# secondlaw-ai/skyrim

Measured on AMD Instinct MI355X. Metric: 6-h forecast steps/sec on 721x1440 state, 1/2/4/8 MI355X; per-channel max rel-err vs ref, higher is better.
Workload: dtype f16; 1 GPU; Pangu 6-h autoregressive rollout, 721x1440x69 state (13 levels x 5 vars + 4 surface), random-init weights (64 M params), state resident in HBM, 1 ensemble membe; parallelism=single GPU, members=1, finite=True, rounding=compensated, term_plan=0x66f

## Files before the change

### skyrim_amd/csrc/attention.hip

```cpp
#include <cstdlib>
#include "gemm_dma.h"
#include "launchers.h"

namespace skp {

__device__ __forceinline__ int attn_key(int f, int row) {
    return f < 8 ? 32 * (f >> 1) + 8 * (row >> 2) + 4 * (f & 1) + (row & 3) : 128 + row;
}

__device__ __forceinline__ void attn_softmax_pv(f32x4 (&s)[9], const uint4 (&vf)[2][5], f32x4 (&o)[2], f32x4& osum) {
    typedef f16 T;
    const float LOG2E = 1.4426950408889634f;
    float mx = s[0][0];
#pragma unroll
    for (int f = 0; f < 9; ++f)
#pragma unroll
        for (int r = 0; r < 4; ++r) mx = fmaxf(mx, s[f][r]);
    mx = fmaxf(mx, __shfl_xor(mx, 16));
    mx = fmaxf(mx, __shfl_xor(mx, 32));
    const float mxl = mx * LOG2E;
#pragma unroll
    for (int f = 0; f < 9; ++f)
#pragma unroll
        for (int r = 0; r < 4; ++r) s[f][r] = __builtin_amdgcn_exp2f(__builtin_fmaf(s[f][r], LOG2E, -mxl));
    o[0] = f32x4{0.f, 0.f, 0.f, 0.f}; o[1] = f32x4{0.f, 0.f, 0.f, 0.f}; osum = f32x4{0.f, 0.f, 0.f, 0.f};
    const uint4 ones = make_uint4(0x3C003C00u, 0x3C003C00u, 0x3C003C00u, 0x3C003C00u);
#pragma unroll
    for (int kb = 0; kb < 5; ++kb) {
        float pv[8];
#pragma unroll
        for (int r = 0; r < 4; ++r) {
            pv[r] = s[2 * kb][r];
            pv[4 + r] = (kb < 4) ? s[(2 * kb + 1) % 9][r] : 0.f;
        }
        uint4 pf[1];
        split8<T, 1>(pv, pf);
#pragma unroll
        for (int df = 0; df < 2; ++df) o[df] = OpT<T>::mfma(as_v8<T>(vf[df][kb]), as_v8<T>(pf[0]), o[df]);
        osum = OpT<T>::mfma(as_v8<T>(ones), as_v8<T>(pf[0]), osum);
    }
}

constexpr int BT_ROW = 28, BT_COPY = 144 * BT_ROW + 120;

template <class TO, int NPL_O>
__global__ void __launch_bounds__(256) __attribute__((amdgpu_waves_per_eu(3, 3))) earth_attention2_kernel(const f16* __restrict__ q, const f16* __restrict__ k,
                                                              const f16* __restrict__ vt, const f16* __restrict__ bias_cmp, TO* __restrict__ out,
                                                              long long out_plane, int ld_out, int nW, int heads) {
    typedef f16 T;
    __shared__ __attribute__((aligned(16))) f16 tabs[4 * BT_COPY];
    const int lane = threadIdx.x & 63, wave = threadIdx.x >> 6;
    const int th = blockIdx.x;
    const int head = th % heads, type = th / heads;
    const int l15 = lane & 15, g = lane >> 4;
    {
        const f16* src = bias_cmp + (long long)th * 3456;
        for (int i = threadIdx.x; i < 3456; i += 256) {
            const int r = i / 24, e = i - 24 * r;
            const f16 v = src[i];
            if (e < 23) {
#pragma unroll
                for (int c = 0; c < 4; ++c) tabs[c * BT_COPY + r * BT_ROW + e + c] = v;
            }
        }
    }
    int koff[9];
#pragma unroll
    for (int f = 0; f < 9; ++f) {
        const int k0 = f < 8 ? 32 * (f >> 1) + 8 * g + 4 * (f & 1) : 128 + 4 * g;
        const int zk = k0 / 72, hk = (k0 / 12) % 6, wk0 = k0 % 12;
        koff[f] = 2 * ((2 * zk * 36 + 6 * hk) * BT_ROW + wk0);
    }
    __syncthreads();
    const char* tb = reinterpret_cast<const char*>(tabs);

    for (int wi = wave; wi < nW; wi += 4) {
        const int win = type * nW + wi;
        const long long base = (long long)win * heads + head;
        const T* qp = q + base * (WIN_TOKENS * HEAD_DIM) + l15 * HEAD_DIM + g * 8;
        const T* kp = k + base * (WIN_TOKENS * HEAD_DIM) + g * 8;
        const T* vp = vt + base * (WIN_TOKENS * HEAD_DIM) + (8 * (l15 >> 2) + (l15 & 3)) * WIN_TOKENS;

        uint4 kf[9];
#pragma unroll
        for (int f = 0; f < 9; ++f) kf[f] = *reinterpret_cast<const uint4*>(kp + attn_key(f, l15) * HEAD_DIM);
        uint4 vf[2][5];
#pragma unroll
        for (int df = 0; df < 2; ++df)
#pragma unroll
            for (int kb = 0; kb < 5; ++kb) {
                const T* s = vp + df * 4 * WIN_TOKENS;
                if (kb < 4) vf[df][kb] = *reinterpret_cast<const uint4*>(s + kb * 32 + g * 8);
                else { const uint2 lo = *reinterpret_cast<const uint2*>(s + 128 + g * 4); vf[df][kb] = make_uint4(lo.x, lo.y, 0, 0); }
            }
        uint4 qn = *reinterpret_cast<const uint4*>(qp);
#pragma unroll 1
        for (int qf = 0; qf < 9; ++qf) {
            const uint4 qv = qn;
            if (qf < 8) qn = *reinterpret_cast<const uint4*>(qp + (qf + 1) * 16 * HEAD_DIM);
            const int qi = 16 * qf + l15;
            const int zq = qi >= 72 ? 1 : 0, hq = (qi - 72 * zq) / 12, wq = qi - 72 * zq - 12 * hq;
            const int c = (wq + 1) & 3;
            const char* bq = tb + 2 * (c * BT_COPY + (zq * 36 + hq) * BT_ROW + (11 - wq) + c);
            uint2 bias[9];
#pragma unroll
            for (int f = 0; f < 9; ++f) bias[f] = *reinterpret_cast<const uint2*>(bq + koff[f]);

            f32x4 s[9];
#pragma unroll
            for (int f = 0; f < 9; ++f) {
                typedef f16 h4 __attribute__((ext_vector_type(4)));
                const h4 b = __builtin_bit_cast(h4, bias[f]);
                s[f] = OpT<T>::mfma(as_v8<T>(kf[f]), as_v8<T>(qv), f32x4{(float)b[0], (float)b[1], (float)b[2], (float)b[3]});
            }
            f32x4 o[2], osum;
            attn_softmax_pv(s, vf, o, osum);
            const float inv = __builtin_amdgcn_rcpf(osum[0]);
            TO* orow = out + blk_off((long long)win * WIN_TOKENS + qf * 16 + l15, head * HEAD_DIM, ld_out) + g * 8;
            const float y[8] = {o[0][0] * inv, o[0][1] * inv, o[0][2] * inv, o[0][3] * inv, o[1][0] * inv, o[1][1] * inv, o[1][2] * inv, o[1][3] * inv};
            store8_planes<TO, NPL_O>(orow, out_plane, y);
        }
    }
}


template <int C_, int PL_>
struct QaShape {
    static constexpr int C = C_, PL = PL_, KS = C / 32, NWAVES = 8, THREADS = 64 * NWAVES;
    static constexpr int BLK_KIB = KS * 2 * PL;
    static constexpr int W_BYTES = 3 * BLK_KIB * 1024;
    static constexpr int TAB_BYTES = (4 * BT_COPY * 2 + 1023) / 1024 * 1024;
    static constexpr int RING_BYTES = 6 * 1024;
    static constexpr int SMEM = W_BYTES + TAB_BYTES + 1024 + NWAVES * RING_BYTES;
    static_assert(SMEM <= 160 * 1024, "LDS");
};

struct QkvAttnArgs {
    const f16* xs;
    const int* widx;
    const f16* wf;
    const float* bias;
    const f16* bias_cmp;
    const f16* zrow;
    f16* out; long long out_plane;
    int nW, heads, types;
    float scale;
};

template <class S, int NPL_O>
__global__ void __launch_bounds__(S::THREADS) __attribute__((amdgpu_waves_per_eu(2, 2)))
qkv_attention_kernel(const QkvAttnArgs a) {
    typedef f16 T;
    constexpr int C = S::C, KS = S::KS, PL = S::PL;
    extern __shared__ __attribute__((aligned(16))) char smem[];
    char* wl = smem;
    f16* tabs = reinterpret_cast<f16*>(smem + S::W_BYTES);
    float* qb = reinterpret_cast<float*>(smem + S::W_BYTES + S::TAB_BYTES);
    const int tid = threadIdx.x, lane = tid & 63, l15 = lane & 15, g = lane >> 4;
    const int wave = __builtin_amdgcn_readfirstlane(tid >> 6);
    const int xcd = blockIdx.x & 7, slot = blockIdx.x >> 3;
    const int head = slot % a.heads, type = xcd + 8 * (slot / a.heads);
    if (type >= a.types) return;
    const int th = type * a.heads + head;
    {
        const unsigned lds_base = (unsigned)(size_t)smem;
#pragma unroll
        for (int which = 0; which < 3; ++which) {
            const f16* src = a.wf + ((long long)(which * a.heads + head) * S::BLK_KIB << 9) + lane * 8;
            for (int p = wave; p < S::BLK_KIB; p += S::NWAVES) glds16(src + (p << 9), lds_base + (unsigned)((which * S::BLK_KIB + p) << 10));
        }
        const f16* src = a.bias_cmp + (long long)th * 3456;
        constexpr int NT = (3456 + S::THREADS - 1) / S::THREADS;
        f16 tv[NT];
#pragma unroll
        for (int j = 0; j < NT; ++j) { const int i = tid + j * S::THREADS; tv[j] = src[i < 3456 ? i : 0]; }
#pragma unroll
        for (int j = 0; j < NT; ++j) {
            const int i = tid + j * S::THREADS;
            const int r = i / 24, e = i - 24 * r;
            if (i < 3456 && e < 23) {
#pragma unroll
                for (int c = 0; c < 4; ++c) tabs[c * BT_COPY + r * BT_ROW + e + c] = tv[j];
            }
        }
        if (tid < 96) qb[tid] = a.bias[(tid >> 5) * C + head * HEAD_DIM + (tid & 31)];
    }
    int koff[9];
#pragma unroll
    for (int f = 0; f < 9; ++f) {
        const int k0 = f < 8 ? 32 * (f >> 1) + 8 * g + 4 * (f & 1) : 128 + 4 * g;
        const int zk = k0 / 72, hk = (k0 / 12) % 6, wk0 = k0 % 12;
        koff[f] = 2 * ((2 * zk * 36 + 6 * hk) * BT_ROW + wk0);
    }
    int srcn[9];
    auto load_src = [&](int wi_) {
        const int w_ = type * a.nW + wi_;
#pragma unroll
        for (int f = 0; f < 9; ++f) srcn[f] = a.widx[w_ * WIN_TOKENS + attn_key(f, l15)];
    };
    load_src(wave < a.nW ? wave : 0);
    asm volatile("s_waitcnt vmcnt(0)" ::: "memory");
    __syncthreads();
    const char* tb = reinterpret_cast<const char*>(tabs);
    const char* wrd = wl + lane * 16;
    const unsigned ring_base = (unsigned)(size_t)smem + (unsigned)(S::W_BYTES + S::TAB_BYTES + 1024 + wave * S::RING_BYTES);
    const char* ring_rd = smem + S::W_BYTES + S::TAB_BYTES + 1024 + wave * S::RING_BYTES + lane * 16;

    for (int wi = wave; wi < a.nW; wi += S::NWAVES) {
        const int win = type * a.nW + wi;
        int src[9];
#pragma unroll
        for (int f = 0; f < 9; ++f) src[f] = srcn[f];
        typedef unsigned u32x9 __attribute__((ext_vector_type(9)));
        u32x9 qx, qy, qz, qw;
        uint4 kf[9];
        uint2 vh[9][2];
        const T* xp[3];
        int xstep[3];
        auto point = [&](int tg_) {
#pragma unroll
            for (int i = 0; i < 3; ++i) {
                const int r = src[3 * tg_ + i];
                xp[i] = r >= 0 ? a.xs + blk_off(r, g * 8, C) : a.zrow;
                xstep[i] = r >= 0 ? 512 : 0;
            }
        };
        auto fetch = [&](int ks) {
#pragma unroll
            for (int i = 0; i < 3; ++i) glds16(xp[i] + ks * xstep[i], ring_base + (unsigned)(((ks & 1) * 3 + i) << 10));
        };
        point(0);
        fetch(0);
        fetch(1);
#pragma unroll
        for (int tg = 0; tg < 3; ++tg) {
            f32x4 qa[3][2], ka[3][2], va[3][2];
#pragma unroll
            for (int i = 0; i < 3; ++i)
#pragma unroll
                for (int n = 0; n < 2; ++n) { qa[i][n] = f32x4{0.f, 0.f, 0.f, 0.f}; ka[i][n] = f32x4{0.f, 0.f, 0.f, 0.f}; va[i][n] = f32x4{0.f, 0.f, 0.f, 0.f}; }
#pragma unroll 1
            for (int ks = 0; ks < KS; ++ks) {
                if (ks + 1 < KS) asm volatile("s_waitcnt vmcnt(3)" ::: "memory");
                else asm volatile("s_waitcnt vmcnt(0)" ::: "memory");
                uint4 xf[3];
#pragma unroll
                for (int i = 0; i < 3; ++i) xf[i] = *reinterpret_cast<const uint4*>(ring_rd + (((ks & 1) * 3 + i) << 10));
                if (ks + 2 < KS) {
                    asm volatile("s_waitcnt lgkmcnt(0)" ::: "memory");
                    fetch(ks + 2);
                }
#pragma unroll
                for (int which = 0; which < 3; ++which)
#pragma unroll
                    for (int n = 0; n < 2; ++n)
#pragma unroll
                        for (int p = PL - 1; p >= 0; --p) {
                            const uint4 w = *reinterpret_cast<const uint4*>(wrd + ((((which * KS + ks) * 2 + n) * PL + p) << 10));
#pragma unroll
                            for (int i = 0; i < 3; ++i) {
                                if (which == 0) qa[i][n] = OpT<T>::mfma(as_v8<T>(w), as_v8<T>(xf[i]), qa[i][n]);
                                else if (which == 1) ka[i][n] = OpT<T>::mfma(as_v8<T>(w), as_v8<T>(xf[i]), ka[i][n]);
                                else va[i][n] = OpT<T>::mfma(as_v8<T>(xf[i]), as_v8<T>(w), va[i][n]);
                            }
                        }
            }
            if (tg < 2) {
                point(tg + 1);
                fetch(0);
                fetch(1);
            }
            float bq[8], bk[8], bv[2];
#pragma unroll
            for (int i = 0; i < 8; ++i) { bq[i] = qb[8 * g + i]; bk[i] = qb[32 + 8 * g + i]; }
#pragma unroll
            for (int df = 0; df < 2; ++df) bv[df] = qb[64 + 8 * (l15 >> 2) + 4 * df + (l15 & 3)];
#pragma unroll
            for (int i = 0; i < 3; ++i) {
                const int f = 3 * tg + i;
                float v[8];
                uint4 o[1];
#pragma unroll
                for (int r = 0; r < 4; ++r) { v[r] = (qa[i][0][r] + bq[r]) * a.scale; v[4 + r] = (qa[i][1][r] + bq[4 + r]) * a.scale; }
                split8<T, 1>(v, o);
                asm volatile("" : "+v"(o[0].x), "+v"(o[0].y), "+v"(o[0].z), "+v"(o[0].w));
                qx[f] = o[0].x; qy[f] = o[0].y; qz[f] = o[0].z; qw[f] = o[0].w;
#pragma unroll
                for (int r = 0; r < 4; ++r) { v[r] = ka[i][0][r] + bk[r]; v[4 + r] = ka[i][1][r] + bk[4 + r]; }
                split8<T, 1>(v, o);
                kf[f] = o[0];
#pragma unroll
                for (int df = 0; df < 2; ++df) {
                    const float u[4] = {va[i][df][0] + bv[df], va[i][df][1] + bv[df], va[i][df][2] + bv[df], va[i][df][3] + bv[df]};
                    uint2 h[1];
                    split4<T, 1>(u, h);
                    vh[f][df] = h[0];
                }
                asm volatile("" : "+v"(kf[f].x), "+v"(kf[f].y), "+v"(kf[f].z), "+v"(kf[f].w), "+v"(vh[f][0].x), "+v"(vh[f][0].y), "+v"(vh[f][1].x), "+v"(vh[f][1].y));
            }
        }
        uint4 vf[2][5];
#pragma unroll
        for (int df = 0; df < 2; ++df) {
#pragma unroll
            for (int kb = 0; kb < 4; ++kb) vf[df][kb] = make_uint4(vh[2 * kb][df].x, vh[2 * kb][df].y, vh[2 * kb + 1][df].x, vh[2 * kb + 1][df].y);
            vf[df][4] = make_uint4(vh[8][df].x, vh[8][df].y, 0, 0);
        }
        if (wi + S::NWAVES < a.nW) load_src(wi + S::NWAVES);
#pragma unroll 1
        for (int qf = 0; qf < 9; ++qf) {
            const uint4 qc = make_uint4(qx[qf], qy[qf], qz[qf], qw[qf]);
            const int qi = attn_key(qf, l15);
            const int zq = qi >= 72 ? 1 : 0, hq = (qi - 72 * zq) / 12, wq = qi - 72 * zq - 12 * hq;
            const int c = (wq + 1) & 3;
            const char* bqp = tb + 2 * (c * BT_COPY + (zq * 36 + hq) * BT_ROW + (11 - wq) + c);
            f32x4 s[9];
#pragma unroll
            for (int f = 0; f < 9; ++f) {
                typedef f16 h4 __attribute__((ext_vector_type(4)));
                const h4 b = __builtin_bit_cast(h4, *reinterpret_cast<const uint2*>(bqp + koff[f]));
                s[f] = OpT<T>::mfma(as_v8<T>(kf[f]), as_v8<T>(qc), f32x4{(float)b[0], (float)b[1], (float)b[2], (float)b[3]});
            }
            f32x4 o[2], osum;
            attn_softmax_pv(s, vf, o, osum);
            const float inv = __builtin_amdgcn_rcpf(osum[0]);
            T* orow = a.out + blk_off((long long)win * WIN_TOKENS + qi, head * HEAD_DIM, C) + g * 8;
            const float y[8] = {o[0][0] * inv, o[0][1] * inv, o[0][2] * inv, o[0][3] * inv, o[1][0] * inv, o[1][1] * inv, o[1][2] * inv, o[1][3] * inv};
            store8_planes<T, NPL_O>(orow, a.out_plane, y);
        }
    }
}

template <class S>
static hipError_t launch_qa(const QkvAttnArgs& a, int types, int out_planes, hipStream_t stream) {
    if (out_planes == 1) {
        auto kern = qkv_attention_kernel<S, 1>;
        hipError_t e = hipFuncSetAttribute(reinterpret_cast<const void*>(kern), hipFuncAttributeMaxDynamicSharedMemorySize, S::SMEM);
        if (e != hipSuccess) return e;
        hipLaunchKernelGGL(kern, dim3((unsigned)(8 * ((types + 7) / 8) * a.heads)), dim3(S::THREADS), S::SMEM, stream, a);
    } else {
        auto kern = qkv_attention_kernel<S, 2>;
        hipError_t e = hipFuncSetAttribute(reinterpret_cast<const void*>(kern), hipFuncAttributeMaxDynamicSharedMemorySize, S::SMEM);
        if (e != hipSuccess) return e;
        hipLaunchKernelGGL(kern, dim3((unsigned)(8 * ((types + 7) / 8) * a.heads)), dim3(S::THREADS), S::SMEM, stream, a);
    }
    return hipGetLastError();
}

hipError_t op_qkv_attention(const Geom& g, const BlockW<f16>& b, const int* widx, int res, const f16* Xs, const Work<PrecF16x3>& wk, hipStream_t s, int out_planes) {
    if (!b.bias_cmp || !(b.qkvh || b.qkvf)) return hipErrorInvalidValue;
    const int heads = res == 0 ? 6 : 12;
    QkvAttnArgs a{Xs, widx, b.qkvh ? b.qkvh : b.qkvf, b.qkv_b, b.bias_cmp, wk.zrow, wk.ao, wk.ao_plane, g.nW[res], heads, g.types[res], 0.17677669529663687f};
    if (b.qkvh) return res == 0 ? launch_qa<QaShape<192, 1>>(a, g.types[res], out_planes, s) : launch_qa<QaShape<384, 1>>(a, g.types[res], out_planes, s);
    if (res != 0) return hipErrorNotSupported;
    return launch_qa<QaShape<192, 2>>(a, g.types[res], out_planes, s);
}

template <class P>
hipError_t launch_attention(const AttnArgs<P>& a, hipStream_t stream) {
    constexpr int NPL_O = (P::NA > P::NW ? P::NA : P::NW);
    const int types = a.n_win / a.nW;
    if (a.out_planes == 1)
        hipLaunchKernelGGL((earth_attention2_kernel<typename P::T, 1>), dim3((unsigned)(types * a.heads)), dim3(256), 0, stream,
                           a.q, a.k, a.vt, a.bias_cmp, a.out, a.out_plane, a.ld_out, a.nW, a.heads);
    else
        hipLaunchKernelGGL((earth_attention2_kernel<typename P::T, NPL_O>), dim3((unsigned)(types * a.heads)), dim3(256), 0, stream,
                           a.q, a.k, a.vt, a.bias_cmp, a.out, a.out_plane, a.ld_out, a.nW, a.heads);
    return hipGetLastError();
}

template hipError_t launch_attention<PrecBF16x3>(const AttnArgs<PrecBF16x3>&, hipStream_t);
template hipError_t launch_attention<PrecF16x3>(const AttnArgs<PrecF16x3>&, hipStream_t);

}
```

Measured before the change: 74.28 steps/s.

## Software-pipeline QKV projection k-loop with register double-buffered LDS fragments

Restructures the fused QKV projection inner k-loop so that weight fragments are prefetched from LDS two MFMA groups ahead in a rotating register ring. Activation fragments are double-buffered in registers, so the next k-step's LDS reads and global-to-LDS fetch overlap the current MFMAs. The k-loop is unrolled by two with compile-time flags for the tail steps, and sched_barriers pin the instruction order. This is meant to hide LDS and global load latency behind matrix-core work, at the cost of more VGPRs and an assumption that KS is even and at least 2.

After: 74.76 steps/s (median of 6 runs). Within noise of the previous version (+0.7%).

```diff
diff --git a/skyrim_amd/csrc/attention.hip b/skyrim_amd/csrc/attention.hip
--- a/skyrim_amd/csrc/attention.hip
+++ b/skyrim_amd/csrc/attention.hip
@@ -1,4 +1,5 @@
 #include <cstdlib>
+#include <type_traits>
 #include "gemm_dma.h"
 #include "launchers.h"
 
@@ -239,32 +240,56 @@
             for (int i = 0; i < 3; ++i)
 #pragma unroll
                 for (int n = 0; n < 2; ++n) { qa[i][n] = f32x4{0.f, 0.f, 0.f, 0.f}; ka[i][n] = f32x4{0.f, 0.f, 0.f, 0.f}; va[i][n] = f32x4{0.f, 0.f, 0.f, 0.f}; }
+            constexpr int NF = 6 * PL, XJ = NF - 2;
+            auto wfrag = [&](int ks, int j) -> uint4 {
+                const int which = j / (2 * PL), n = (j / PL) & 1, p = PL - 1 - j % PL;
+                return *reinterpret_cast<const uint4*>(wrd + ((((which * KS + ks) * 2 + n) * PL + p) << 10));
+            };
+            uint4 xa[3], xb[3], wr[3];
+            auto kstep = [&](auto f2, auto f1, int ks, uint4 (&cur)[3], uint4 (&nxt)[3]) {
+                constexpr bool F2 = decltype(f2)::value, F1 = decltype(f1)::value;
+                if (F2) {
+                    asm volatile("" :: "v"(cur[0].w), "v"(cur[1].w), "v"(cur[2].w));
+                    fetch(ks + 2);
+                    __builtin_amdgcn_sched_barrier(0);
+                }
+#pragma unroll
+                for (int j = 0; j < NF; ++j) {
+                    if (F1 && j == XJ) {
+                        if (F2) asm volatile("s_waitcnt vmcnt(3)" ::: "memory");
+                        else asm volatile("s_waitcnt vmcnt(0)" ::: "memory");
+#pragma unroll
+                        for (int i = 0; i < 3; ++i) nxt[i] = *reinterpret_cast<const uint4*>(ring_rd + ((((ks + 1) & 1) * 3 + i) << 10));
+                    }
+                    if (j + 2 < NF) wr[(j + 2) % 3] = wfrag(ks, j + 2);
+                    else if (F1) wr[(j + 2) % 3] = wfrag(ks + 1, j + 2 - NF);
+                    __builtin_amdgcn_sched_barrier(0);
+                    const uint4 w = wr[j % 3];
+                    const int which = j / (2 * PL), n = (j / PL) & 1;
+#pragma unroll
+                    for (int i = 0; i < 3; ++i) {
+                        if (which == 0) qa[i][n] = OpT<T>::mfma(as_v8<T>(w), as_v8<T>(cur[i]), qa[i][n]);
+                        else if (which == 1) ka[i][n] = OpT<T>::mfma(as_v8<T>(w), as_v8<T>(cur[i]), ka[i][n]);
+                        else va[i][n] = OpT<T>::mfma(as_v8<T>(cur[i]), as_v8<T>(w), va[i][n]);
+                    }
+                    __builtin_amdgcn_sched_barrier(0);
+                }
+            };
+            asm volatile("s_waitcnt vmcnt(3)" ::: "memory");
+#pragma unroll
+            for (int i = 0; i < 3; ++i) xa[i] = *reinterpret_cast<const uint4*>(ring_rd + (i << 10));
+            wr[0] = wfrag(0, 0);
+            wr[1] = wfrag(0, 1);
+            __builtin_amdgcn_sched_barrier(0);
+            constexpr std::true_type yes{};
+            constexpr std::false_type no{};
 #pragma unroll 1
-            for (int ks = 0; ks < KS; ++ks) {
-                if (ks + 1 < KS) asm volatile("s_waitcnt vmcnt(3)" ::: "memory");
-                else asm volatile("s_waitcnt vmcnt(0)" ::: "memory");
-                uint4 xf[3];
-#pragma unroll
-                for (int i = 0; i < 3; ++i) xf[i] = *reinterpret_cast<const uint4*>(ring_rd + (((ks & 1) * 3 + i) << 10));
-                if (ks + 2 < KS) {
-                    asm volatile("s_waitcnt lgkmcnt(0)" ::: "memory");
-                    fetch(ks + 2);
-                }
-#pragma unroll
-                for (int which = 0; which < 3; ++which)
-#pragma unroll
-                    for (int n = 0; n < 2; ++n)
-#pragma unroll
-                        for (int p = PL - 1; p >= 0; --p) {
-                            const uint4 w = *reinterpret_cast<const uint4*>(wrd + ((((which * KS + ks) * 2 + n) * PL + p) << 10));
-#pragma unroll
-                            for (int i = 0; i < 3; ++i) {
-                                if (which == 0) qa[i][n] = OpT<T>::mfma(as_v8<T>(w), as_v8<T>(xf[i]), qa[i][n]);
-                                else if (which == 1) ka[i][n] = OpT<T>::mfma(as_v8<T>(w), as_v8<T>(xf[i]), ka[i][n]);
-                                else va[i][n] = OpT<T>::mfma(as_v8<T>(xf[i]), as_v8<T>(w), va[i][n]);
-                            }
-                        }
-            }
+            for (int ks = 0; ks + 2 < KS; ks += 2) {
+                kstep(yes, yes, ks, xa, xb);
+                kstep(yes, yes, ks + 1, xb, xa);
+            }
+            kstep(no, yes, KS - 2, xa, xb);
+            kstep(no, no, KS - 1, xb, xa);
             if (tg < 2) {
                 point(tg + 1);
                 fetch(0);
```
